# Roestlab/diffusion-deconvolution-dia-msms-data

Measured on AMD Instinct MI355X. Metric: MS2 windows/s (train step: zero_grad + train_step + backward + clip 10 + AdamW), higher is better.
Workload: dtype f32; 1 GPU; BASELINE configs[1]: default UNet1d (dim 4, mults 1,2,2,3,3,4,4; 128,847 params), synthetic MS2+MS1 windows 400 RT x 64 m/z, batch 32 per GPU, fp32; global_batch=32, parallelism=dp1

## Files before the change

diffusion-deconvolution-dia-msms-data_amd/csrc/dq_kernels.h:

```cpp
#pragma once
#include <hip/hip_runtime.h>
#include <cstdint>

namespace dq {

constexpr int MSE_MAX_BLOCKS = 1024;

int launch_q_sample(const float* alpha_bars, const float* x0, const int64_t* t, const float* noise, float* x_t, int B,
                    int64_t per_sample, int normalize, hipStream_t s);
int launch_sample_finish(const float* x, const float* ms2_cond, float* out_x, float* out_noise, int64_t n, int normalize,
                         hipStream_t s);
int launch_mse_fwd_bwd(const float* eps, const float* noise, float* loss_out, float* grad_out, float* partials, int64_t n,
                       hipStream_t s, const float* lw = nullptr, const int64_t* t = nullptr, int64_t per_sample = 0, float tm = 1.f,
                       float ta = 0.f, int* defer_sum = nullptr);
int launch_sum_partials(const float* partials, int count, float scale, float* out, hipStream_t s);
int launch_ms1_loss(const float* out, const float* x_t, const float* ms1, float cm, float ca, const float* lw, const int64_t* t, float w,
                    int B, int RT, int MZ, float* grad, float* loss_out, float* scratch, hipStream_t s);
constexpr int MSE_PW_SLICE = 8192;
int64_t mse_per_window_scratch_bytes(int B, int64_t per);
int launch_mse_per_window(const float* out, const float* target, float tm, float ta, const float* lw, const int64_t* t, float* per_window,
                          float* loss_out, void* scratch, int64_t scratch_bytes, int B, int64_t per, hipStream_t s);
int launch_axpy(float* dst, const float* src, int64_t n, hipStream_t s);
int launch_zero(float* dst, int64_t n, hipStream_t s);
int launch_copy(float* dst, const float* src, int64_t n, hipStream_t s);
// ... 247 lines not shown
struct ConvBwdWg {
  const float* dy = nullptr;
  const float* in = nullptr;
  const float* w = nullptr;
  float* din = nullptr; int accumulate = 0;
  float* part = nullptr; int64_t part_floats = 0;
  float* dparams = nullptr;
  int C = 0, pre = 0, cp = 0, rows = 0, n = 0, rows_per_sample = 1;
  int tiles_ps = 0, tpb = 0, nv = 0;
};
bool conv_wg_usable(int C, int pre, int cp, int n, int rows_per_sample);
int64_t conv_wg_part_floats(int C, int pre, int cp, int B, int rows_per_sample, int n);
int launch_conv_bwd_wg(const ConvBwdWg& a, hipStream_t s, ResWgReduce* red_out);
inline PartReduce res_part_reduce(const float* gpart, int gx, int B, int C, float* dg2, float* dg1, float* dss, int ss_stride) {
  PartReduce r;
  r.part = gpart; r.B = B; r.gx = gx; r.nv = 4 * C; r.nseg = 2;
  r.seg_start[0] = 0; r.seg_len[0] = C; r.seg_dst[0] = dg2;
  r.seg_start[1] = C; r.seg_len[1] = C; r.seg_dst[1] = dg1;
  r.s0 = 2 * C; r.sn = 2 * C; r.sdst = dss; r.sstride = ss_stride;
  return r;
}

int launch_rmsnorm_fwd(const float* x, const float* g, float* y, int C, int rows, int n, hipStream_t s);

int launch_fold(const float* in, float* out, int B, int RT, int cn, int to_mid, int add, hipStream_t s, int pitch = 0);

int launch_prep_inputs(const float* x, const float* cond, const float* ms1, const float* ss, int ss_stride, int ss_off, float cm,
                       float ca, float* cat0, float* ms1n, int B, int RT, int MZ, hipStream_t s);
int launch_ms1_norm(const float* ms1, float cm, float ca, float* ms1n, int64_t n, hipStream_t s);
constexpr int MS1_MAX_CHANNELS = 4096;
constexpr int MS1_FWD_TP = 8, MS1_FWD_WAVES = 4;
constexpr int MS1_WG_T = 64, MS1_WG_MAX_PARTS = 256;
struct Ms1FeatFwd {
  const float* ms1 = nullptr;
  const float* w = nullptr; const float* bias = nullptr;
  float cm = 1.f, ca = 0.f;
  float* ms1n_out = nullptr;
  float* u_out = nullptr;
  float* a_out = nullptr;
  int B = 0, RT = 0, M1 = 0;
};
int launch_ms1_feat_fwd(const Ms1FeatFwd& a, hipStream_t s);
struct Ms1FeatWgrad {
  const float* ms1n = nullptr; const float* du = nullptr;
  float* dw = nullptr; float* dbias = nullptr;
  float* part = nullptr; int64_t part_floats = 0;
  int B = 0, RT = 0, M1 = 0;
};
int ms1_feat_wgrad_parts(int B, int RT, int M1);
int64_t ms1_feat_wgrad_part_floats(int B, int RT, int M1);
int launch_ms1_feat_wgrad(const Ms1FeatWgrad& a, hipStream_t s);
int launch_prep_inputs_bwd(const float* dcat0, const float* cond, float cm, float ca, float* dss, int ss_stride, int ss_off, int B,
                           int RT, int MZ, float* part, int64_t part_floats, hipStream_t s);

int launch_im2col3(const float* x, float* xcol, int B, int C, int RT, int P, hipStream_t s);
int launch_col2im3(const float* dxcol, float* dx, int B, int C, int RT, int P, int accumulate, hipStream_t s);
int launch_repitch(float* dst, int dpitch, const float* src, int spitch, int64_t rows, int n, hipStream_t s);
int launch_zero_pads(float* x, int64_t rows, int RT, int P, hipStream_t s);
int launch_wnorm_fwd(const float* u, const float* g, const float* ss, int ss_stride, int act, const float* res, float* y, int B, int C,
                     int RT, int P, hipStream_t s);
int launch_wnorm_bwd(const float* u, const float* dy, const float* g, const float* ss, int ss_stride, int act, float* du, float* dg,
                     float* dss, float* dbias, float* scratch, int B, int C, int RT, int P, hipStream_t s);
int launch_rowsum(const float* x, int64_t rows, int RT, int P, float* out, hipStream_t s);
int launch_sum_b(const float* part, int B, int C, float* dst, hipStream_t s);


struct LinAttn {
  const float* x = nullptr; float* y = nullptr;
  const float* w_qkv = nullptr; const float* w_out = nullptr; const float* b_out = nullptr;
  const float* g_pre = nullptr; const float* g_out = nullptr;
  int C = 0, rows = 0, n = 0;
  float* ypre = nullptr;
  const float* prep = nullptr;
};
inline bool la_short_row(int n) { return n <= 64 && (n & (n - 1)) == 0; }
enum LaFwdForm { LA_FWD_LONG, LA_FWD_SMALL, LA_FWD_ROWS, LA_FWD_REG };
LaFwdForm la_fwd_form(const LinAttn& a);
int launch_linattn_fwd(const LinAttn& a, hipStream_t s);
bool la_small_usable(int C, int n);
int la_small_min_rows();
int launch_la_small_fwd(const LinAttn& a, hipStream_t s);
struct LinAttnBwd;
bool la_rows_bwd_usable(int C, int n);
int la_rows_bwd_min_rows();
bool la_rows_fwd_usable(int C, int n);
int launch_la_rows_fwd(const LinAttn& a, hipStream_t s);
int launch_la_rows_bwd(const LinAttnBwd& a, int max_slots, int* slots_out, hipStream_t s);
constexpr int LA_PREP_BOUNDED = 1024 + 4096;
constexpr int LA_PREP_BF16 = 1024 + 4096 + 8;
constexpr int LA_PREP_SMALL = 1024 + 4096 + 8 + 6144;
constexpr int LA_ROWS_LANE_FLOATS = 36;
constexpr int LA_PREP_ROWS = 1024 + 4096 + 8 + 6144 + 6144;
constexpr int LA_PREP_FLOATS = LA_PREP_ROWS + 4 * 64 * LA_ROWS_LANE_FLOATS;
struct LaPrepItem { const float* w_qkv; const float* w_out; int C; float* prep; const float* g_pre; };
constexpr int LA_PREP_MAX = 16;
struct PrepCopy { const float* src; float* dst; int n; };
constexpr int PREP_COPY_MAX = 4;
int launch_linattn_prepare(const LaPrepItem* items, int count, hipStream_t s, const PrepCopy* copies = nullptr, int n_copies = 0);
struct LinAttnBwd {
  LinAttn f;
  const float* dy = nullptr; float* dx = nullptr;
  int dx_store = 0;
  const float* ypre = nullptr;
  float* dyp = nullptr; float* dxh = nullptr;
  float* part = nullptr; int64_t part_floats = 0;
  int defer_reduce = 0; int* waves_out = nullptr;
// ... 33 lines not shown
```

diffusion-deconvolution-dia-msms-data_amd/csrc/dq_unet.hip:

```cpp
#include "dq_dev.h"
#include "dq_tfm.h"
#include "dq_ops.h"
#include "dq_options.h"
#include "../../include/dq_hip.h"

#include <algorithm>
#include <functional>
#include <cmath>
#include <cstdlib>
#include <cstring>
#include <vector>

namespace dq {

void layout_arena(const Plan& p, int B, int RT, Arena& a) {
  int64_t zero_total = 0;
  for (int pass = 0; pass < 2; ++pass) {
  a = Arena();
  a.B = B; a.RT = RT;
  int64_t off = 0, off_nz = zero_total;
  auto take = [&](int64_t n) { int64_t o = off; off += (n + 63) / 64 * 64; return o; };
  auto take_nz = [&](int64_t n) { int64_t o = off_nz; off_nz += (n + 63) / 64 * 64; return o; };
  const int64_t R = (int64_t)B * RT;
  auto res = [&](int rows_per_sample, int cin, int c, int n, bool zero_out = false) {
// ... 735 lines not shown
      DQ_TRY(tiny_bwd_run(c, tiny_bwd_desc(c, true, lp.tb_up_w), true));
    } else {
      DQ_TRY(la_bwd(c, l.la, b, c.w(b.r1.out), c.g(b.la), c.g(b.r1.out), R, l.n, lp.prep_ok ? L + ui : -1));
      DQ_TRY(res_bwd(c, l.r1, b.r1, c.w(b.r0.out), c.g(b.r0.out), cx, c.w(a.downs[lv].r0.out), c.g(a.downs[lv].r0.out), cs, R, l.n, RT, 1, 1));
      DQ_TRY(res_bwd(c, l.r0, b.r0, c.w(in_off), c.g(in_off), cx, c.w(a.downs[lv].la), c.g(a.downs[lv].la), cs, R, l.n, RT, 1, 1));
    }
    if (side_flush_here(lv)) DQ_TRY(side_flush(c));
  }
  if (p.wide_mid) {
    DQ_TRY(mid_backward_wide(c, rope));
  } else {
    if (!lp.use_tb_up) DQ_TRY(launch_fold(c.g(a.mid_back), c.g(a.mid2.out), B, RT, p.mid_c, 1, 1, c.s));
    DQ_TRY(mid_backward(c, rope, grad_x != nullptr, lp.prep_ok));
    if (!lp.use_tb_dn) DQ_TRY(launch_fold(c.g(a.mid_in), c.g(a.downs[L - 1].rs), B, RT, p.mid_c, 0, 0, c.s));
  }
  auto ms1_bwd = [&p, &a, B, RT](const Ctx& cc) -> int {
    DQ_TRY(conv_plain_bwd(cc, p.ms1_c1, CONV_S1, cc.w(a.ms1_a), cc.g(a.ms1f), cc.g(a.ms1_a), B, RT, RT, 0));
    BlockBwd gb;
    gb.u = cc.w(a.ms1_u); gb.dy = cc.g(a.ms1_a); gb.du = cc.g(a.ms1_u); gb.C = p.cond_dim; gb.rows = B; gb.n = RT; gb.rows_per_sample = 1;
    gb.act = ACT_GELU;
    DQ_TRY(launch_block_bwd(gb, cc.s));
    if (p.ms1_channels > 1) {
      Ms1FeatWgrad w;
      w.ms1n = cc.w(a.ms1n); w.du = cc.g(a.ms1_u); w.dw = cc.dprm(p.ms1_c0.w); w.dbias = cc.dprm(p.ms1_c0.b);
      w.part = cc.w(a.ms1_wpart); w.part_floats = a.ms1_wpart_floats; w.B = B; w.RT = RT; w.M1 = p.ms1_channels;
      return launch_ms1_feat_wgrad(w, cc.s);
    }
    return conv_plain_bwd(cc, p.ms1_c0, CONV_S1, cc.w(a.ms1n), cc.g(a.ms1_u), nullptr, B, RT, RT, 0);
  };
  DQ_TRY(on_side(c, tail_fork_enabled(), ms1_bwd));
  for (int lv = L - 1; lv >= 0; --lv) {
    const LevelP& l = p.downs[lv];
    const LevelBuf& b = a.downs[lv];
    const int C = l.r0.cin;
    const int64_t in_off = lv == 0 ? a.h0 : a.downs[lv - 1].rs;
    if (lv == L - 1 && lp.use_tb_dn) {
      DQ_TRY(tiny_bwd_run(c, tiny_bwd_desc(c, false, false), false));
      if (side_flush_here(lv)) DQ_TRY(side_flush(c));
      continue;
    }
    if (!(lv == L - 2 && lp.use_tb_dn))
      DQ_TRY(resample_bwd(c, l.resample, l.last ? LEVEL_PRE_S1 : LEVEL_PRE_DOWN, b, l.n, l.n_next, 1));
    if (lv == 0) DQ_TRY(side_flush(c));
    DQ_TRY(la_bwd(c, l.la, b, c.w(b.r1.out), c.g(b.la), c.g(b.r1.out), R, l.n, lp.prep_ok ? lv : -1));
    DQ_TRY(res_bwd(c, l.r1, b.r1, c.w(b.r0.out), c.g(b.r0.out), C, nullptr, nullptr, 0, R, l.n, RT));
    if (lv == 0) DQ_TRY(side_flush(c));
    DQ_TRY(res_bwd(c, l.r0, b.r0, c.w(in_off), c.g(in_off), C, nullptr, nullptr, 0, R, l.n, RT, lv > 0 ? 1 : 0, 0));
    if (lv == 2 && p.mz <= 64) {
      DQ_TRY(la_flush_side(c));
      DQ_TRY(wg_to_side());
    }
    if (side_flush_here(lv)) DQ_TRY(side_flush(c));
  }
  auto init_bwd = [&p, &a, init_cond, cm, ca, B, RT, R](const Ctx& cc) -> int {
    DQ_TRY(conv_plain_bwd(cc, p.init_conv, CONV_S1, cc.w(a.cat0), cc.g(a.h0), cc.g(a.cat0), R, p.mz, p.mz, 0));
    return launch_prep_inputs_bwd(cc.g(a.cat0), init_cond, cm, ca, cc.g(a.ss), p.ss_total, p.ss_init, B, RT, p.mz, cc.w(a.bb_part),
                                  a.bb_part_floats, cc.s);
  };
  const bool tail_swap = !DQ_DEV_FLAG("DQ_NO_TAIL_SWAP", '1');
  if (side_open(c, tail_swap && !grad_x && tail_fork_enabled())) {
    DQ_TRY(side_flush(c));
    hipEvent_t ev_ss = nullptr;
    if (c.owner->side_used) DQ_TRY(side_mark(c, &ev_ss));
    DQ_TRY(conv_plain_bwd(c, p.init_conv, CONV_S1, c.w(a.cat0), c.g(a.h0), nullptr, R, p.mz, p.mz, 0));
    DQ_TRY(la_flush_side(c));
    DQ_TRY(side_flush(c));
    DQ_TRY(conv_plain_bwd(c, p.init_conv, CONV_S1, c.w(a.cat0), c.g(a.h0), c.g(a.cat0), R, p.mz, p.mz, 0, -1, false));
    if (ev_ss) DQ_HIP_OK(hipStreamWaitEvent(c.s, ev_ss, 0));
    DQ_TRY(launch_prep_inputs_bwd(c.g(a.cat0), init_cond, cm, ca, c.g(a.ss), p.ss_total, p.ss_init, B, RT, p.mz, c.w(a.bb_part), a.bb_part_floats,
                                  c.s));
    DQ_TRY(la_flush(c));
    DQ_TRY(res_wg_reduce_all(wg_items, c.s));
    DQ_TRY(launch_time_embed_bwd(p, dt, c.P, c.dP, c.w(a.tbuf), c.g(a.ss), B, c.s));
    return join_side(c);
  }
  DQ_TRY(on_side(c, !grad_x && tail_fork_enabled(), init_bwd));
  if (grad_x) {
    DQ_HIP_OK(hipMemcpy2DAsync(grad_x, sizeof(float) * p.mz, c.g(a.cat0) + p.mz, sizeof(float) * 2 * p.mz, sizeof(float) * p.mz, R,
                               hipMemcpyDeviceToDevice, c.s));
  }
  DQ_TRY(bwd_close(c, queues));
  return launch_time_embed_bwd(p, dt, c.P, c.dP, c.w(a.tbuf), c.g(a.ss), B, c.s);
}

int unet_sample_prologue(const Ctx& c, const float* ms1, float cm, float ca, const float* rope, bool* ran) {
  const Plan& p = c.p;
  const Arena& a = c.ar;
  *ran = false;
  if (p.wide_mid) return 0;
  const LevelPlan lp = level_plan(p, a, c.B, c.RT, false, false);
  DQ_TRY(unet_prepare(c, lp, c.s));
  DQ_TRY(ms1_features(c, ms1, cm, ca, true, c.s));
  DQ_TRY(conv_plain_fwd(c, proj(p.k_w, HID, p.cond_dim), CONV_S1, c.w(a.ms1f), c.w(a.kk), c.B, c.RT, c.RT, lp.prep_ok ? 1 : -1));
  if (rope) DQ_TRY(launch_rope(c.w(a.kk), rope, c.B, (int64_t)HID * c.RT, c.RT, 1.f, c.s));
  *ran = true;
  return 0;
}

int ensure_arena(dq_plan* plan, int B, int RT) {
  if (plan->arena.B != B || plan->arena.RT != RT) layout_arena(plan->plan, B, RT, plan->arena);
  if (!plan->dev.ss_w_off) {
    const Plan& p = plan->plan;
    std::vector<int64_t> woff(p.ss_total), boff(p.ss_total);
    for (const auto& l : p.ss_lins)
      for (int r = 0; r < l.rows; ++r) {
        woff[l.ss_off + r] = l.w + (int64_t)r * p.time_dim;
        boff[l.ss_off + r] = l.b + r;
      }
    DQ_HIP_OK(hipMalloc(&plan->dev.ss_w_off, sizeof(int64_t) * p.ss_total));
    DQ_HIP_OK(hipMalloc(&plan->dev.ss_b_off, sizeof(int64_t) * p.ss_total));
    DQ_HIP_OK(hipMemcpy(plan->dev.ss_w_off, woff.data(), sizeof(int64_t) * p.ss_total, hipMemcpyHostToDevice));
    DQ_HIP_OK(hipMemcpy(plan->dev.ss_b_off, boff.data(), sizeof(int64_t) * p.ss_total, hipMemcpyHostToDevice));
  }
  return 0;
}

}

using namespace dq;

extern "C" {

int dq_debug_level_plan(dq_plan* plan, int B, int RT, int save, int twin, int32_t* out, int cap) {
// ... 163 lines not shown
```

diffusion-deconvolution-dia-msms-data_amd/csrc/k_conv.hip:

```cpp
#include "dq_common.h"
#include "dq_kernels.h"
#include <cstdlib>

namespace dq {

template <int MODE, int K>
__device__ __forceinline__ int tap_pos(int p, int k, int n_in) {
  if (MODE == CONV_S1) {
    const int q = p + k - (K - 1) / 2;
    return (q >= 0 && q < n_in) ? q : -1;
  } else if (MODE == CONV_DOWN) {
    const int q = 2 * p + k - 1;
    return (q >= 0 && q < n_in) ? q : -1;
  } else {
    const int j = p + k - 1;
    return (j >= 0 && j < 2 * n_in) ? (j >> 1) : -1;
  }
}

template <int COUT, int K, int MODE>
__global__ void __launch_bounds__(256) k_conv_fwd(ConvFwd a) {
  const int64_t item = blockIdx.x * (int64_t)blockDim.x + threadIdx.x;
  const int64_t total = (int64_t)a.rows * a.n_out;
  const int co_base = blockIdx.y * COUT;
// ... 950 lines not shown
    const int b = (int)(i / ((int64_t)RT * cn));
    const int64_t src = ((int64_t)b * cn + c) * P + rt;
    out[i] = add ? out[i] + in[src] : in[src];
  }
}

int launch_fold(const float* in, float* out, int B, int RT, int cn, int to_mid, int add, hipStream_t s, int pitch) {
  const int P = pitch > 0 ? pitch : RT;
  const int64_t total = (int64_t)B * (to_mid ? P : RT) * cn;
  if (total == 0) return 0;
  hipLaunchKernelGGL(k_fold, dim3(cdiv(total, 256)), dim3(256), 0, s, in, out, B, RT, cn, to_mid, add, P);
  DQ_LAUNCH_CHECK();
  return 0;
}

__global__ void __launch_bounds__(256) k_prep_inputs(const float* __restrict__ x, const float* __restrict__ cond,
                                                     const float* __restrict__ ms1, const float* __restrict__ ss, int ss_stride,
                                                     int ss_off, float cm, float ca, float* __restrict__ cat0,
                                                     float* __restrict__ ms1n, int B, int RT, int MZ) {
  const int64_t i = blockIdx.x * (int64_t)blockDim.x + threadIdx.x;
  const int64_t total = (int64_t)B * RT * MZ;
  if (ms1n && i < (int64_t)B * RT) ms1n[i] = fmaf(ms1[i], cm, ca);
  if (i >= total) return;
  const int mz = (int)(i % MZ);
  const int64_t row = i / MZ;
  const int b = (int)(row / RT);
  const float sc = ss[(int64_t)b * ss_stride + ss_off], sh = ss[(int64_t)b * ss_stride + ss_off + 1];
  const float cn = fmaf(cond[i], cm, ca);
  cat0[(row * 2 + 0) * MZ + mz] = cn * (sc + 1.0f) + sh;
  cat0[(row * 2 + 1) * MZ + mz] = x[i];
}

int launch_prep_inputs(const float* x, const float* cond, const float* ms1, const float* ss, int ss_stride, int ss_off, float cm,
                       float ca, float* cat0, float* ms1n, int B, int RT, int MZ, hipStream_t s) {
  const int64_t total = (int64_t)B * RT * MZ;
  if (total == 0) return 0;
  hipLaunchKernelGGL(k_prep_inputs, dim3(cdiv(total, 256)), dim3(256), 0, s, x, cond, ms1, ss, ss_stride, ss_off, cm, ca, cat0,
                     ms1n, B, RT, MZ);
  DQ_LAUNCH_CHECK();
  return 0;
}

__global__ void __launch_bounds__(256) k_ms1_norm(const float* __restrict__ ms1, float cm, float ca, float* __restrict__ ms1n, int64_t n) {
  const int64_t i = blockIdx.x * (int64_t)blockDim.x + threadIdx.x;
  if (i < n) ms1n[i] = fmaf(ms1[i], cm, ca);
}
int launch_ms1_norm(const float* ms1, float cm, float ca, float* ms1n, int64_t n, hipStream_t s) {
  if (n == 0) return 0;
  hipLaunchKernelGGL(k_ms1_norm, dim3(cdiv(n, 256)), dim3(256), 0, s, ms1, cm, ca, ms1n, n);
  DQ_LAUNCH_CHECK();
  return 0;
}

__global__ void __launch_bounds__(256) k_prep_inputs_bwd(const float* __restrict__ dcat0, const float* __restrict__ cond, float cm,
                                                         float ca, float* __restrict__ part, int RT, int MZ) {
  const int b = blockIdx.y;
  const int64_t per = (int64_t)RT * MZ;
  float dsc = 0.f, dsh = 0.f;
  for (int64_t it = blockIdx.x * (int64_t)blockDim.x + threadIdx.x; it < per; it += (int64_t)gridDim.x * blockDim.x) {
    const int mz = (int)(it % MZ);
    const int64_t row = (int64_t)b * RT + it / MZ;
    const float d = dcat0[(row * 2 + 0) * MZ + mz];
    dsh += d;
    dsc = fmaf(d, fmaf(cond[(int64_t)b * per + it], cm, ca), dsc);
  }
  __shared__ float red[4][2];
  dsc = wave_sum(dsc);
  dsh = wave_sum(dsh);
  if ((threadIdx.x & 63) == 0) { red[threadIdx.x >> 6][0] = dsc; red[threadIdx.x >> 6][1] = dsh; }
  __syncthreads();
  if (threadIdx.x < 2)
    part[((int64_t)b * gridDim.x + blockIdx.x) * 2 + threadIdx.x] =
        (red[0][threadIdx.x] + red[1][threadIdx.x]) + (red[2][threadIdx.x] + red[3][threadIdx.x]);
}

int launch_prep_inputs_bwd(const float* dcat0, const float* cond, float cm, float ca, float* dss, int ss_stride, int ss_off, int B,
                           int RT, int MZ, float* part, int64_t part_floats, hipStream_t s) {
  const int64_t per = (int64_t)RT * MZ;
  if (per == 0 || B == 0) return 0;
  dim3 grid(std::max(1, std::min(32, cdiv(per, 1024))), B);
  DQ_REQUIRE(part && part_floats >= (int64_t)grid.x * B * 2, "prep_inputs_bwd: partial-sum slot missing or too small");
  hipLaunchKernelGGL(k_prep_inputs_bwd, grid, dim3(256), 0, s, dcat0, cond, cm, ca, part, RT, MZ);
  DQ_LAUNCH_CHECK();
  PartReduce r;
  r.part = part; r.B = B; r.gx = (int)grid.x; r.nv = 2; r.s0 = 0; r.sn = 2; r.sdst = dss + ss_off; r.sstride = ss_stride;
  return launch_part_reduce(r, s);
}

}
```

diffusion-deconvolution-dia-msms-data_amd/csrc/k_res_wg.hip:

```cpp
#include "dq_common.h"
#include "dq_kernels.h"
#include "k_res_common.h"
#include "dq_probe.h"
#include <algorithm>

namespace dq {

namespace {

typedef float f32x4 __attribute__((ext_vector_type(4)));
__device__ __forceinline__ f32x4 mfma4(float a, float b, f32x4 c) { return __builtin_amdgcn_mfma_f32_4x4x1f32(a, b, c, 0, 0, 0); }

__device__ __forceinline__ float lane_m1(float v) { return __int_as_float(__builtin_amdgcn_mov_dpp(__float_as_int(v), 0x138, 0xF, 0xF, true)); }
__device__ __forceinline__ float lane_p1(float v) { return __int_as_float(__builtin_amdgcn_mov_dpp(__float_as_int(v), 0x130, 0xF, 0xF, true)); }
constexpr int pad4(int x) { return (x + 3) / 4 * 4; }

constexpr int TILE = 256;
constexpr int RUN = 16;

template <int C>
struct Img {
  static constexpr int ST = C == 4 ? 4 : 12;
  static constexpr int FLOATS = (TILE + 2) * ST + ((TILE + 2) / RUN + 1) * 4;
  __device__ static __forceinline__ int at(int q) { return q * ST + (q >> 4) * 4; }
};
template <int ST>
__device__ __forceinline__ constexpr int run_off(int s) { return s * ST + (s == RUN - 1 ? 4 : 0); }


}

template <int C, bool WR>
__global__ void __launch_bounds__(256, 2) k_res_bwd_wg(ResBwdWg a) {
  using I = Img<C>;
  constexpr int ST = I::ST, CQ = C / 4;
  extern __shared__ __attribute__((aligned(16))) float lds_all[];
  float* i_du2 = lds_all;
  float* i_du1 = i_du2 + I::FLOATS;
  float* i_a1 = i_du1 + I::FLOATS;
  float* i_xa = i_a1 + I::FLOATS;
  float* i_xb = i_xa + I::FLOATS;
  float* i_do = i_xb + (WR ? I::FLOATS : 4);
  float (*red)[4 * C] = reinterpret_cast<float (*)[4 * C]>(i_do + (WR ? I::FLOATS : 4));
  constexpr int GI = WR ? 2 * CQ : CQ;
  constexpr int JT2 = C * CQ * 3, JT1 = C * GI * 3, JTR = WR ? C * GI : 0;
  constexpr int OT1 = pad4(JT2), OTR = OT1 + pad4(JT1), JTT = OTR + pad4(JTR);
  float* wl = reinterpret_cast<float*>(red) + 4 * 4 * C;
  float* prm = wl + JTT * 4;
  const int cin = a.cinA + a.cinB;
  DQ_PSTAMP(100000 + C * 10 + (WR ? 1 : 0), 0);
  for (int idx = threadIdx.x; idx < JTT * 4; idx += 256) {
    const int j = (idx >> 4) * 4 + (idx & 3), l4 = (idx >> 2) & 3;
    float v = 0.f;
    if (j < JT2) {
      const int k = j % 3, gg = (j / 3) % CQ, co = j / (3 * CQ);
      v = a.w2[(co * C + 4 * gg + l4) * 3 + k];
    } else if (j >= OT1 && j < OT1 + JT1) {
      const int jj = j - OT1, k = jj % 3, gi = (jj / 3) % GI, co = jj / (3 * GI), ci = 4 * gi + l4;
      if (ci < cin) v = a.w1[(co * cin + ci) * 3 + k];
    } else if (WR && j >= OTR && j < OTR + JTR) {
      const int jj = j - OTR, gi = jj % GI, co = jj / GI, ci = 4 * gi + l4;
      if (ci < cin) v = a.wr[co * cin + ci];
    }
    wl[idx] = v;
  }
  for (int i = threadIdx.x; i < 4 * C; i += 256) {
    const int what = i / C, c = i % C;
    const float* ssp = a.ss + (int64_t)blockIdx.y * a.ss_stride;
    prm[i] = what == 0 ? a.g2[c] : what == 1 ? a.g1[c] : what == 2 ? ssp[c] : ssp[C + c];
  }
  __syncthreads();
  DQ_PSTAMP(100000 + C * 10 + (WR ? 1 : 0), 1);
  const int b = blockIdx.y, n = a.n;
  const int per_sample = a.rows_per_sample * n;
  const int tid = threadIdx.x, lane = tid & 63;
  const int wv = __builtin_amdgcn_readfirstlane(tid >> 6);
  const int q = tid + 1;
  const int blk = lane >> 2, li = lane & 3;
  const int lb = I::at(blk * RUN + 1) + li;
  const bool n8 = n == 8;
  const bool zl = ((blk * RUN) % n) == 0;
  const bool zr = ((blk * RUN + RUN) % n) == 0;
  const int cinq = cin >> 2;
  const int g = C == 8 ? (wv & 1) : 0, hs = C == 8 ? (wv >> 1) : wv;
  const bool doW2 = C == 8 ? true : wv == 0;
  const int hW2 = C == 8 ? hs : 0;
  const bool doB2 = C == 8 ? hs == 0 : wv == 0;
  const bool doWr = WR && (C == 8 ? true : wv == 1);
  const int hr0 = C == 8 ? 2 * hs : 0, hr1 = C == 8 ? 2 * hs + 1 : 1;
  const bool doBr = WR && (C == 8 ? hs == 0 : wv == 1);
  const bool doW1 = C == 8 ? true : (wv == 2 || (WR && wv == 3));
  const int h10 = C == 8 ? (WR ? 2 * hs : hs) : (wv == 3 ? 1 : 0);
  const int h11 = (C == 8 && WR) ? 2 * hs + 1 : -1;
  const bool doB1 = C == 8 ? hs == 0 : wv == 2;
  const bool v_r0 = doWr && hr0 < cinq, v_r1 = doWr && hr1 < cinq;
  const bool v_10 = doW1 && h10 < cinq, v_11 = doW1 && h11 >= 0 && h11 < cinq;
  auto ximg = [&](int h) -> const float* { return (h < CQ || !WR ? i_xa + 4 * (h < CQ ? h : 0) : i_xb + 4 * (h - CQ)) + lb; };

  f32x4 aW2[1][3], aWr[2], aW1[2][3], aB2 = {0.f, 0.f, 0.f, 0.f}, aBr = aB2, aB1 = aB2;
#pragma unroll
  for (int h = 0; h < 1; ++h)
#pragma unroll
    for (int k = 0; k < 3; ++k) aW2[h][k] = aB2;
#pragma unroll
  for (int h = 0; h < 2; ++h) {
#pragma unroll
    for (int k = 0; k < 3; ++k) aW1[h][k] = aB2;
    aWr[h] = aB2;
  }
  float dg2[C], dg1[C], dsc[C], dsh[C];
#pragma unroll
  for (int c = 0; c < C; ++c) dg2[c] = dg1[c] = dsc[c] = dsh[c] = 0.f;
  const float sqC = sqrtf((float)C);
  const float* wlane = wl + li * 4;
  auto wop = [&](int j) -> float { return wlane[(j >> 2) * 16 + (j & 3)]; };

  const int tile_end = min(a.tiles_ps, ((int)blockIdx.x + 1) * a.tpb);
#pragma unroll 1
  for (int tile = blockIdx.x * a.tpb; tile < tile_end; ++tile) {
    const int it = tile * TILE + tid;
    const bool live = it < per_sample;
    const int itc = live ? it : per_sample - 1;
    const int row = b * a.rows_per_sample + itc / n, p = itc % n;
    const unsigned boA = (((unsigned)row * C) * (unsigned)n + (unsigned)p) * 4u;
    const unsigned boB = (((unsigned)row * (unsigned)a.cinB) * (unsigned)n + (unsigned)p) * 4u;
    auto ld = [&](const float* base, int c, unsigned boff) -> float {
      return *reinterpret_cast<const float*>(reinterpret_cast<const char*>(base + (size_t)c * n) + boff);
    };
    auto st = [&](float* base, int c, unsigned boff, float v) {
      *reinterpret_cast<float*>(reinterpret_cast<char*>(base + (size_t)c * n) + boff) = v;
    };
    const bool hasL = live && p > 0, hasR = live && p + 1 < n;
    float dout[C], d[C], u[C], u1v[C], xa[C], xb[WR ? C : 1];
#pragma unroll
    for (int c = 0; c < C; ++c) {
      dout[c] = ld(a.dout, c, boA);
      u[c] = ld(a.u2, c, boA);
      u1v[c] = ld(a.u1, c, boA);
      xa[c] = ld(a.inA, c, boA);
    }
    if constexpr (WR) {
#pragma unroll
      for (int c = 0; c < C; ++c) xb[c] = c < a.cinB ? ld(a.inB, c, boB) : 0.f;
    }
#pragma unroll
    for (int c = 0; c < C; ++c) { dout[c] = live ? dout[c] : 0.f; d[c] = dout[c]; }
    norm_act_bwd<C, false>(u, d, prm, nullptr, dg2, nullptr, nullptr);
    float a1v[C];
    {
      float ssq = 0.f;
#pragma unroll
      for (int c = 0; c < C; ++c) ssq = fmaf(u1v[c], u1v[c], ssq);
      const float inv = rms_inv(ssq, sqC);
#pragma unroll
      for (int c = 0; c < C; ++c) a1v[c] = silu_f(fmaf(u1v[c] * inv * prm[C + c], prm[2 * C + c] + 1.0f, prm[3 * C + c]));
    }
    DQ_PSTAMP(100000 + C * 10 + (WR ? 1 : 0), 2);
    __syncthreads();
    {
      const int o = I::at(q);
#pragma unroll
      for (int c4 = 0; c4 < CQ; ++c4) {
        const int c = 4 * c4;
        *reinterpret_cast<float4*>(i_du2 + o + c) = live ? make_float4(d[c], d[c + 1], d[c + 2], d[c + 3]) : make_float4(0.f, 0.f, 0.f, 0.f);
        *reinterpret_cast<float4*>(i_a1 + o + c) = make_float4(a1v[c], a1v[c + 1], a1v[c + 2], a1v[c + 3]);
        *reinterpret_cast<float4*>(i_xa + o + c) = make_float4(xa[c], xa[c + 1], xa[c + 2], xa[c + 3]);
        if constexpr (WR) {
          *reinterpret_cast<float4*>(i_xb + o + c) = make_float4(xb[c], xb[c + 1], xb[c + 2], xb[c + 3]);
          *reinterpret_cast<float4*>(i_do + o + c) = make_float4(dout[c], dout[c + 1], dout[c + 2], dout[c + 3]);
        }
      }
    }
    __syncthreads();
    DQ_PSTAMP(100000 + C * 10 + (WR ? 1 : 0), 3);
    if (doW2) {
      const float* A = i_du2 + lb + 4 * g;
      const float* Bp = i_a1 + lb + 4 * hW2;
      float bprev = zl ? 0.f : Bp[-ST], bcur = Bp[0];
#pragma unroll
      for (int s = 0; s < RUN; ++s) {
        const float av = A[run_off<ST>(s)];
        float bnext = s + 1 < RUN ? Bp[run_off<ST>(s + 1 < RUN ? s + 1 : s)] : (zr ? 0.f : Bp[RUN * ST + 4]);
        float b0 = bprev, b2 = bnext;
        if (s == 8) b0 = n8 ? 0.f : b0;
        if (s == 7) b2 = n8 ? 0.f : b2;
        aW2[0][0] = mfma4(av, b0, aW2[0][0]);
        aW2[0][1] = mfma4(av, bcur, aW2[0][1]);
        aW2[0][2] = mfma4(av, b2, aW2[0][2]);
        aB2 = mfma4(av, 1.f, aB2);
        bprev = bcur; bcur = bnext;
      }
    }
    if constexpr (WR) {
     if (doWr) {
      const float* A = i_do + lb + 4 * g;
      const float* X0 = ximg(hr0);
// ... 75 lines not shown
    }
    DQ_PSTAMP(100000 + C * 10 + (WR ? 1 : 0), 8);
    if (a.dA || a.dB) {
#pragma unroll
      for (int pass = 0; pass < (WR ? 2 : 1); ++pass) {
        f32x4 acc[CQ][3], ar[CQ];
#pragma unroll
        for (int q4 = 0; q4 < CQ; ++q4) {
#pragma unroll
          for (int k = 0; k < 3; ++k) acc[q4][k] = f32x4{0.f, 0.f, 0.f, 0.f};
          ar[q4] = f32x4{0.f, 0.f, 0.f, 0.f};
        }
#pragma unroll
        for (int co = 0; co < C; ++co) {
          const float dc = live ? da1[co] : 0.f;
          const float tp = lane_p1(dc), tm = lane_m1(dc);
          const float dr = hasR ? tp : 0.f, dl = hasL ? tm : 0.f;
#pragma unroll
          for (int q4 = 0; q4 < CQ; ++q4) {
            const int gi = pass * CQ + q4;
            const int j = OT1 + (co * GI + gi) * 3;
            acc[q4][0] = mfma4(wop(j + 0), dr, acc[q4][0]);
            acc[q4][1] = mfma4(wop(j + 1), dc, acc[q4][1]);
            acc[q4][2] = mfma4(wop(j + 2), dl, acc[q4][2]);
            if constexpr (WR) ar[q4] = mfma4(wop(OTR + co * GI + gi), dout[co], ar[q4]);
          }
        }
        if (pass == 0) DQ_PSTAMP(100000 + C * 10 + (WR ? 1 : 0), 11);
        float v[C];
#pragma unroll
        for (int q4 = 0; q4 < CQ; ++q4)
#pragma unroll
          for (int i = 0; i < 4; ++i) v[4 * q4 + i] = (acc[q4][0][i] + acc[q4][1][i]) + (acc[q4][2][i] + (WR ? ar[q4][i] : dout[4 * q4 + i]));
        if (pass == 0) {
          if (live && a.dA) {
            float oldv[C];
#pragma unroll
            for (int c = 0; c < C; ++c) oldv[c] = 0.f;
            if (!a.dA_store) {
#pragma unroll
              for (int c = 0; c < C; ++c) oldv[c] = ld(a.dA, c, boA);
            }
            DQ_PSTAMP(100000 + C * 10 + (WR ? 1 : 0), 12);
#pragma unroll
            for (int c = 0; c < C; ++c) st(a.dA, c, boA, oldv[c] + v[c]);
          }
        } else {
          if (live && a.dB) {
            float oldv[C];
#pragma unroll
            for (int c = 0; c < C; ++c) oldv[c] = 0.f;
            if (!a.dB_store) {
#pragma unroll
              for (int c = 0; c < C; ++c) oldv[c] = c < a.cinB ? ld(a.dB, c, boB) : 0.f;
            }
#pragma unroll
            for (int c = 0; c < C; ++c)
              if (c < a.cinB) st(a.dB, c, boB, oldv[c] + v[c]);
          }
        }
      }
    }
    DQ_PSTAMP(100000 + C * 10 + (WR ? 1 : 0), 9);
  }

  float* part = a.part + ((int64_t)blockIdx.y * gridDim.x + blockIdx.x) * a.nv;
  const int oC1W = 0, oC1B = C * cin * 3, oG1 = oC1B + C, oC2W = oG1 + C, oC2B = oC2W + C * C * 3, oG2 = oC2B + C, oRW = oG2 + C,
            oRB = oRW + C * cin, nglob = WR ? oRB + C : oRW;
  auto put_w = [&](f32x4 acc, int base, int h, int kdim, int k, int ld) {
    const f32x4 t = blocks_sum(acc);
    if (lane < 4) {
#pragma unroll
      for (int i = 0; i < 4; ++i) part[base + ((4 * g + i) * ld + 4 * h + lane) * kdim + k] = t[i];
    }
  };
  auto put_b = [&](f32x4 acc, int base) {
    const f32x4 t = blocks_sum(acc);
    if (lane == 0) {
#pragma unroll
      for (int i = 0; i < 4; ++i) part[base + 4 * g + i] = t[i];
    }
  };
  if (doW2) {
#pragma unroll
    for (int k = 0; k < 3; ++k) put_w(aW2[0][k], oC2W, hW2, 3, k, C);
  }
  if (doB2) put_b(aB2, oC2B);
  if (v_r0) put_w(aWr[0], oRW, hr0, 1, 0, cin);
  if (v_r1) put_w(aWr[1], oRW, hr1, 1, 0, cin);
  if (doBr) put_b(aBr, oRB);
  if (v_10) {
#pragma unroll
    for (int k = 0; k < 3; ++k) put_w(aW1[0][k], oC1W, h10, 3, k, cin);
  }
  if (v_11) {
#pragma unroll
    for (int k = 0; k < 3; ++k) put_w(aW1[1][k], oC1W, h11, 3, k, cin);
  }
  if (doB1) put_b(aB1, oC1B);
#pragma unroll
  for (int c = 0; c < C; ++c) {
    const float s0 = wave_sum(dg2[c]), s1 = wave_sum(dg1[c]), s2 = wave_sum(dsc[c]), s3 = wave_sum(dsh[c]);
    if (lane == 0) { red[wv][c] = s0; red[wv][C + c] = s1; red[wv][2 * C + c] = s2; red[wv][3 * C + c] = s3; }
  }
  __syncthreads();
  for (int i = tid; i < 4 * C; i += 256) {
    const float v = (red[0][i] + red[1][i]) + (red[2][i] + red[3][i]);
    const int what = i / C, c = i % C;
    part[(what == 0 ? oG2 : what == 1 ? oG1 : what == 2 ? nglob : nglob + C) + c] = v;
  }
  DQ_PSTAMP(100000 + C * 10 + (WR ? 1 : 0), 10);
}

__global__ void __launch_bounds__(256) k_res_wg_reduce(ResWgReduceMulti m) {
  const ResWgReduce& r = m.it[blockIdx.y];
  const int twoC = 2 * r.C;
  const int nelem = r.nglob + r.B * twoC;
// ... 22 lines not shown
    if (k < cnt) s0 += src[(int64_t)k * r.nv];
  }
  red[gq][el] = s0 + s1;
  __syncthreads();
  if (gq == 0 && e < nelem) {
    float s = 0.f;
#pragma unroll
    for (int k = 0; k < 16; ++k) s += red[k][el];
    if (e < r.nglob) r.dst[e] += s;
    else r.dss[(int64_t)((e - r.nglob) / twoC) * r.ss_stride + (e - r.nglob) % twoC] += s;
  }
}

bool res_wg_usable(int n, int C, int cinA, int cinB, int rows_per_sample) {
  if (!(C == 4 || C == 8)) return false;
  return n >= 8 && n <= 64 && (n & (n - 1)) == 0 && rows_per_sample > 1 && cinA == C && (cinB == 0 || (cinB % 4 == 0 && cinB <= C));
}

template <int C, bool WR>
static size_t res_wg_lds_bytes() {
  constexpr int CQ = C / 4, GI = WR ? 2 * CQ : CQ;
  constexpr int JT2 = C * CQ * 3, JT1 = C * GI * 3, JTR = WR ? C * GI : 0;
  constexpr int JTT = pad4(JT2) + pad4(JT1) + pad4(JTR);
  return sizeof(float) * ((size_t)(WR ? 6 : 4) * Img<C>::FLOATS + (WR ? 0 : 8) + 16 * C + (size_t)JTT * 4 + 4 * C);
}

void res_wg_grid(int B, int rows_per_sample, int n, int* tiles_ps, int* tpb, int* gx) {
  *tiles_ps = cdiv((int64_t)rows_per_sample * n, TILE);
  const int64_t total = (int64_t)*tiles_ps * B;
  *tpb = (int)std::max<int64_t>(1, (total + 1023) / 1024);
  *gx = cdiv(*tiles_ps, *tpb);
}
int res_wg_nv(int C, int cin, bool wr) { return C * cin * 3 + C + C + C * C * 3 + C + C + (wr ? C * cin + C : 0) + 2 * C; }
int64_t res_wg_part_floats(int C, int cin, bool wr, int B, int rows_per_sample, int n) {
  int tiles_ps, tpb, gx;
  res_wg_grid(B, rows_per_sample, n, &tiles_ps, &tpb, &gx);
  return (int64_t)gx * B * res_wg_nv(C, cin, wr);
}

int launch_res_bwd_wg(const ResBwdWg& a_in, hipStream_t s, ResWgReduce* red_out) {
  ResBwdWg a = a_in;
  DQ_REQUIRE(res_wg_usable(a.n, a.C, a.cinA, a.cinB, a.rows_per_sample), "res_bwd_wg: unsupported shape");
  DQ_REQUIRE(a.rows % a.rows_per_sample == 0, "res_bwd_wg: rows must be a multiple of rows_per_sample");
  DQ_REQUIRE((int64_t)a.rows * a.C * a.n * 4 < (1ll << 32), "res_bwd_wg: tensors of 4 GB or more are not built (32-bit byte offsets)");
  DQ_REQUIRE(a.wr || a.cinB == 0, "res_bwd_wg: identity residual needs C input channels");
  DQ_REQUIRE(a.dout && a.u1 && a.u2 && a.inA && (a.cinB == 0 || a.inB) && a.w1 && a.w2 && a.g1 && a.g2 && a.ss && a.part,
             "res_bwd_wg: missing operand");
  const int B = a.rows / a.rows_per_sample;
  int gx;
  res_wg_grid(B, a.rows_per_sample, a.n, &a.tiles_ps, &a.tpb, &gx);
  const bool wr = a.wr != nullptr;
  const void* fn = nullptr;
  size_t lds = 0;
#define DQ_WGK(CC, WW) if (a.C == CC && wr == WW) { fn = (const void*)k_res_bwd_wg<CC, WW>; lds = res_wg_lds_bytes<CC, WW>(); }
  DQ_WGK(4, true) DQ_WGK(4, false) DQ_WGK(8, true) DQ_WGK(8, false)
#undef DQ_WGK
  DQ_REQUIRE(fn && lds <= 160 * 1024, "res_bwd_wg: no kernel for this shape");
  {
    static int occ[2][2] = {{0, 0}, {0, 0}};
    int& o = occ[a.C / 4 - 1][wr];
    if (!o) {
      if (lds > 48 * 1024) DQ_HIP_OK(hipFuncSetAttribute(fn, hipFuncAttributeMaxDynamicSharedMemorySize, (int)lds));
      int nb = 0;
      DQ_HIP_OK(hipOccupancyMaxActiveBlocksPerMultiprocessor(&nb, fn, 256, lds));
      o = std::max(1, std::min(nb, 6));
    }
    int dev = 0;
    hipDeviceProp_t pr;
    static const int cus = (hipGetDevice(&dev) == hipSuccess && hipGetDeviceProperties(&pr, dev) == hipSuccess) ? pr.multiProcessorCount : 256;
    const int64_t resident = (int64_t)o * cus, total = (int64_t)a.tiles_ps * B;
    a.tpb = std::max(a.tpb, (int)((total + resident - 1) / resident));
    while (a.tpb < a.tiles_ps && (int64_t)cdiv(a.tiles_ps, a.tpb) * B > resident) ++a.tpb;
    gx = cdiv(a.tiles_ps, a.tpb);
  }
  a.nv = res_wg_nv(a.C, a.cinA + a.cinB, wr);
  DQ_REQUIRE(a.part_floats >= (int64_t)gx * B * a.nv, "res_bwd_wg: slot scratch too small");
  dim3 grid(gx, B), block(256);
#define DQ_WGL(CC, WW) if (a.C == CC && wr == WW) hipLaunchKernelGGL((k_res_bwd_wg<CC, WW>), grid, block, lds, s, a);
  DQ_WGL(4, true) DQ_WGL(4, false) DQ_WGL(8, true) DQ_WGL(8, false)
#undef DQ_WGL
  DQ_LAUNCH_CHECK();
  if (red_out) {
    ResWgReduce r;
    r.part = a.part; r.B = B; r.gx = gx; r.nv = a.nv; r.nglob = a.nv - 2 * a.C; r.C = a.C;
    r.dst = a.dparams; r.dss = a.dss; r.ss_stride = a.ss_stride;
    *red_out = r;
  }
  return 0;
}

int launch_res_wg_reduce(const ResWgReduce* items, int count, hipStream_t s) {
  if (count == 0) return 0;
  DQ_REQUIRE(count <= RES_WG_REDUCE_MAX, "res_wg_reduce: too many items");
  ResWgReduceMulti m;
  int nmax = 1;
  for (int i = 0; i < count; ++i) {
    m.it[i] = items[i];
    DQ_REQUIRE(items[i].part && items[i].dst && items[i].dss, "res_wg_reduce: missing operand");
    nmax = std::max(nmax, items[i].nglob + items[i].B * 2 * items[i].C);
  }
  hipLaunchKernelGGL(k_res_wg_reduce, dim3(cdiv(nmax, 16), count), dim3(256), 0, s, m);
  DQ_LAUNCH_CHECK();
  return 0;
}

}
```

Before: 10220 windows/s.

## Fuse init-conv input-grad into cond-scale reduction; specialize res wgrad kernel on row length

Adds a kernel that computes the init convolution's input gradient on the fly inside the conditioning scale/shift reduction, so the dcat0 gradient tensor is no longer written and reread. Separately templates the residual weight-gradient kernel on the row length N, which turns the div/mod into compile-time shifts, precomputes byte offsets, splits full and tail tiles, and raises launch-bounds occupancy for C=4. These are unrelated ideas bundled together. The cost is more template instantiations and a recomputed convolution whose inner loop over output channels is less parallel.

Result: no change. 10160 windows/s (-0.5%).

```diff
diff --git a/diffusion-deconvolution-dia-msms-data_amd/csrc/dq_kernels.h b/diffusion-deconvolution-dia-msms-data_amd/csrc/dq_kernels.h
--- a/diffusion-deconvolution-dia-msms-data_amd/csrc/dq_kernels.h
+++ b/diffusion-deconvolution-dia-msms-data_amd/csrc/dq_kernels.h
@@ -323,6 +323,9 @@
 int launch_ms1_feat_wgrad(const Ms1FeatWgrad& a, hipStream_t s);
 int launch_prep_inputs_bwd(const float* dcat0, const float* cond, float cm, float ca, float* dss, int ss_stride, int ss_off, int B,
                            int RT, int MZ, float* part, int64_t part_floats, hipStream_t s);
+bool init_cond_bwd_usable(int cout, int K, int mode);
+int launch_init_cond_bwd(const float* dh0, const float* w, int cout, int cin, const float* cond, float cm, float ca, float* dss,
+                         int ss_stride, int ss_off, int B, int RT, int MZ, float* part, int64_t part_floats, hipStream_t s);
 
 int launch_im2col3(const float* x, float* xcol, int B, int C, int RT, int P, hipStream_t s);
 int launch_col2im3(const float* dxcol, float* dx, int B, int C, int RT, int P, int accumulate, hipStream_t s);
diff --git a/diffusion-deconvolution-dia-msms-data_amd/csrc/dq_unet.hip b/diffusion-deconvolution-dia-msms-data_amd/csrc/dq_unet.hip
--- a/diffusion-deconvolution-dia-msms-data_amd/csrc/dq_unet.hip
+++ b/diffusion-deconvolution-dia-msms-data_amd/csrc/dq_unet.hip
@@ -811,10 +811,18 @@
     }
     if (side_flush_here(lv)) DQ_TRY(side_flush(c));
   }
-  auto init_bwd = [&p, &a, init_cond, cm, ca, B, RT, R](const Ctx& cc) -> int {
-    DQ_TRY(conv_plain_bwd(cc, p.init_conv, CONV_S1, cc.w(a.cat0), cc.g(a.h0), cc.g(a.cat0), R, p.mz, p.mz, 0));
+  const bool fuse_cond = !grad_x && init_cond_bwd_usable(p.init_conv.cout, p.init_conv.k, CONV_S1);
+  auto cond_bwd = [&p, &a, init_cond, cm, ca, B, RT, R, fuse_cond](const Ctx& cc) -> int {
+    if (fuse_cond)
+      return launch_init_cond_bwd(cc.g(a.h0), cc.prm(p.init_conv.w), p.init_conv.cout, p.init_conv.cin, init_cond, cm, ca, cc.g(a.ss),
+                                  p.ss_total, p.ss_init, B, RT, p.mz, cc.w(a.bb_part), a.bb_part_floats, cc.s);
+    DQ_TRY(conv_plain_bwd(cc, p.init_conv, CONV_S1, cc.w(a.cat0), cc.g(a.h0), cc.g(a.cat0), R, p.mz, p.mz, 0, -1, false));
     return launch_prep_inputs_bwd(cc.g(a.cat0), init_cond, cm, ca, cc.g(a.ss), p.ss_total, p.ss_init, B, RT, p.mz, cc.w(a.bb_part),
                                   a.bb_part_floats, cc.s);
+  };
+  auto init_bwd = [&p, &a, R, cond_bwd](const Ctx& cc) -> int {
+    DQ_TRY(conv_plain_bwd(cc, p.init_conv, CONV_S1, cc.w(a.cat0), cc.g(a.h0), nullptr, R, p.mz, p.mz, 0));
+    return cond_bwd(cc);
   };
   const bool tail_swap = !DQ_DEV_FLAG("DQ_NO_TAIL_SWAP", '1');
   if (side_open(c, tail_swap && !grad_x && tail_fork_enabled())) {
@@ -824,10 +832,8 @@
     DQ_TRY(conv_plain_bwd(c, p.init_conv, CONV_S1, c.w(a.cat0), c.g(a.h0), nullptr, R, p.mz, p.mz, 0));
     DQ_TRY(la_flush_side(c));
     DQ_TRY(side_flush(c));
-    DQ_TRY(conv_plain_bwd(c, p.init_conv, CONV_S1, c.w(a.cat0), c.g(a.h0), c.g(a.cat0), R, p.mz, p.mz, 0, -1, false));
     if (ev_ss) DQ_HIP_OK(hipStreamWaitEvent(c.s, ev_ss, 0));
-    DQ_TRY(launch_prep_inputs_bwd(c.g(a.cat0), init_cond, cm, ca, c.g(a.ss), p.ss_total, p.ss_init, B, RT, p.mz, c.w(a.bb_part), a.bb_part_floats,
-                                  c.s));
+    DQ_TRY(cond_bwd(c));
     DQ_TRY(la_flush(c));
     DQ_TRY(res_wg_reduce_all(wg_items, c.s));
     DQ_TRY(launch_time_embed_bwd(p, dt, c.P, c.dP, c.w(a.tbuf), c.g(a.ss), B, c.s));
diff --git a/diffusion-deconvolution-dia-msms-data_amd/csrc/k_conv.hip b/diffusion-deconvolution-dia-msms-data_amd/csrc/k_conv.hip
--- a/diffusion-deconvolution-dia-msms-data_amd/csrc/k_conv.hip
+++ b/diffusion-deconvolution-dia-msms-data_amd/csrc/k_conv.hip
@@ -1026,6 +1026,17 @@
   return 0;
 }
 
+__device__ __forceinline__ void prep_inputs_flush(float dsc, float dsh, float* __restrict__ part) {
+  __shared__ float red[4][2];
+  dsc = wave_sum(dsc);
+  dsh = wave_sum(dsh);
+  if ((threadIdx.x & 63) == 0) { red[threadIdx.x >> 6][0] = dsc; red[threadIdx.x >> 6][1] = dsh; }
+  __syncthreads();
+  if (threadIdx.x < 2)
+    part[((int64_t)blockIdx.y * gridDim.x + blockIdx.x) * 2 + threadIdx.x] =
+        (red[0][threadIdx.x] + red[1][threadIdx.x]) + (red[2][threadIdx.x] + red[3][threadIdx.x]);
+}
+
 __global__ void __launch_bounds__(256) k_prep_inputs_bwd(const float* __restrict__ dcat0, const float* __restrict__ cond, float cm,
                                                          float ca, float* __restrict__ part, int RT, int MZ) {
   const int b = blockIdx.y;
@@ -1038,27 +1049,73 @@
     dsh += d;
     dsc = fmaf(d, fmaf(cond[(int64_t)b * per + it], cm, ca), dsc);
   }
-  __shared__ float red[4][2];
-  dsc = wave_sum(dsc);
-  dsh = wave_sum(dsh);
-  if ((threadIdx.x & 63) == 0) { red[threadIdx.x >> 6][0] = dsc; red[threadIdx.x >> 6][1] = dsh; }
+  prep_inputs_flush(dsc, dsh, part);
+}
+
+constexpr int INIT_TAIL_K = 7, INIT_TAIL_WMAX = 1024;
+__global__ void __launch_bounds__(256) k_init_cond_bwd(const float* __restrict__ du, const float* __restrict__ w, int cout, int cin,
+                                                       const float* __restrict__ cond, float cm, float ca, float* __restrict__ part,
+                                                       int RT, int MZ) {
+  constexpr int K = INIT_TAIL_K;
+  __shared__ float wsh[INIT_TAIL_WMAX];
+  for (int i = threadIdx.x; i < cout * K; i += 256) wsh[i] = w[(int64_t)(i / K) * cin * K + i % K];
   __syncthreads();
-  if (threadIdx.x < 2)
-    part[((int64_t)b * gridDim.x + blockIdx.x) * 2 + threadIdx.x] =
-        (red[0][threadIdx.x] + red[1][threadIdx.x]) + (red[2][threadIdx.x] + red[3][threadIdx.x]);
+  const int b = blockIdx.y;
+  const int64_t per = (int64_t)RT * MZ;
+  float dsc = 0.f, dsh = 0.f;
+  for (int64_t it = blockIdx.x * (int64_t)blockDim.x + threadIdx.x; it < per; it += (int64_t)gridDim.x * blockDim.x) {
+    const int mz = (int)(it % MZ);
+    const int64_t row = (int64_t)b * RT + it / MZ;
+    float acc = 0.f;
+    for (int co = 0; co < cout; ++co) {
+      const float* dup = du + (row * cout + co) * MZ;
+      float dv[K];
+#pragma unroll
+      for (int k = 0; k < K; ++k) {
+        const int p = mz - k + (K - 1) / 2;
+        dv[k] = (p >= 0 && p < MZ) ? dup[p] : 0.f;
+      }
+#pragma unroll
+      for (int k = 0; k < K; ++k) acc = fmaf(wsh[co * K + k], dv[k], acc);
+    }
+    const float d = 0.f + acc;
+    dsh += d;
+    dsc = fmaf(d, fmaf(cond[(int64_t)b * per + it], cm, ca), dsc);
+  }
+  prep_inputs_flush(dsc, dsh, part);
+}
+
+namespace {
+dim3 prep_inputs_grid(int64_t per, int B) { return dim3(std::max(1, std::min(32, cdiv(per, 1024))), B); }
+int prep_inputs_reduce(float* part, int B, int gx, float* dss, int ss_stride, int ss_off, hipStream_t s) {
+  PartReduce r;
+  r.part = part; r.B = B; r.gx = gx; r.nv = 2; r.s0 = 0; r.sn = 2; r.sdst = dss + ss_off; r.sstride = ss_stride;
+  return launch_part_reduce(r, s);
+}
 }
 
 int launch_prep_inputs_bwd(const float* dcat0, const float* cond, float cm, float ca, float* dss, int ss_stride, int ss_off, int B,
                            int RT, int MZ, float* part, int64_t part_floats, hipStream_t s) {
   const int64_t per = (int64_t)RT * MZ;
   if (per == 0 || B == 0) return 0;
-  dim3 grid(std::max(1, std::min(32, cdiv(per, 1024))), B);
+  const dim3 grid = prep_inputs_grid(per, B);
   DQ_REQUIRE(part && part_floats >= (int64_t)grid.x * B * 2, "prep_inputs_bwd: partial-sum slot missing or too small");
   hipLaunchKernelGGL(k_prep_inputs_bwd, grid, dim3(256), 0, s, dcat0, cond, cm, ca, part, RT, MZ);
   DQ_LAUNCH_CHECK();
-  PartReduce r;
-  r.part = part; r.B = B; r.gx = (int)grid.x; r.nv = 2; r.s0 = 0; r.sn = 2; r.sdst = dss + ss_off; r.sstride = ss_stride;
-  return launch_part_reduce(r, s);
-}
-
-}
+  return prep_inputs_reduce(part, B, (int)grid.x, dss, ss_stride, ss_off, s);
+}
+
+bool init_cond_bwd_usable(int cout, int K, int mode) { return K == INIT_TAIL_K && mode == CONV_S1 && cout > 0 && cout * K <= INIT_TAIL_WMAX; }
+int launch_init_cond_bwd(const float* dh0, const float* w, int cout, int cin, const float* cond, float cm, float ca, float* dss,
+                         int ss_stride, int ss_off, int B, int RT, int MZ, float* part, int64_t part_floats, hipStream_t s) {
+  const int64_t per = (int64_t)RT * MZ;
+  if (per == 0 || B == 0) return 0;
+  DQ_REQUIRE(dh0 && w && cond && cin > 0 && init_cond_bwd_usable(cout, INIT_TAIL_K, CONV_S1), "init_cond_bwd: missing operand or unsupported conv");
+  const dim3 grid = prep_inputs_grid(per, B);
+  DQ_REQUIRE(part && part_floats >= (int64_t)grid.x * B * 2, "init_cond_bwd: partial-sum slot missing or too small");
+  hipLaunchKernelGGL(k_init_cond_bwd, grid, dim3(256), 0, s, dh0, w, cout, cin, cond, cm, ca, part, RT, MZ);
+  DQ_LAUNCH_CHECK();
+  return prep_inputs_reduce(part, B, (int)grid.x, dss, ss_stride, ss_off, s);
+}
+
+}
diff --git a/diffusion-deconvolution-dia-msms-data_amd/csrc/k_res_wg.hip b/diffusion-deconvolution-dia-msms-data_amd/csrc/k_res_wg.hip
--- a/diffusion-deconvolution-dia-msms-data_amd/csrc/k_res_wg.hip
+++ b/diffusion-deconvolution-dia-msms-data_amd/csrc/k_res_wg.hip
@@ -3,6 +3,7 @@
 #include "k_res_common.h"
 #include "dq_probe.h"
 #include <algorithm>
+#include <type_traits>
 
 namespace dq {
 
@@ -30,10 +31,12 @@
 
 }
 
-template <int C, bool WR>
-__global__ void __launch_bounds__(256, 2) k_res_bwd_wg(ResBwdWg a) {
+template <int C, bool WR, int N>
+__global__ void __launch_bounds__(256, (C == 4 && !(WR && N <= 16)) ? 4 : 2) k_res_bwd_wg(ResBwdWg a) {
+  static_assert(N == 8 || N == 16 || N == 32 || N == 64, "rows of 8, 16, 32 or 64 positions");
   using I = Img<C>;
   constexpr int ST = I::ST, CQ = C / 4;
+  constexpr int LOGN = N == 8 ? 3 : N == 16 ? 4 : N == 32 ? 5 : 6;
   extern __shared__ __attribute__((aligned(16))) float lds_all[];
   float* i_du2 = lds_all;
   float* i_du1 = i_du2 + I::FLOATS;
@@ -71,16 +74,24 @@
   }
   __syncthreads();
   DQ_PSTAMP(100000 + C * 10 + (WR ? 1 : 0), 1);
-  const int b = blockIdx.y, n = a.n;
-  const int per_sample = a.rows_per_sample * n;
+  const int b = blockIdx.y;
+  const int per_sample = a.rows_per_sample * N;
   const int tid = threadIdx.x, lane = tid & 63;
   const int wv = __builtin_amdgcn_readfirstlane(tid >> 6);
   const int q = tid + 1;
   const int blk = lane >> 2, li = lane & 3;
   const int lb = I::at(blk * RUN + 1) + li;
-  const bool n8 = n == 8;
-  const bool zl = ((blk * RUN) % n) == 0;
-  const bool zr = ((blk * RUN + RUN) % n) == 0;
+  constexpr bool n8 = N == 8;
+  const bool zl = ((blk * RUN) % N) == 0;
+  const bool zr = ((blk * RUN + RUN) % N) == 0;
+  auto inB_has = [&](int c) -> bool { return (c & ~3) < a.cinB; };
+  const int p = tid & (N - 1);
+  const bool hasLp = p > 0, hasRp = p + 1 < N;
+  const unsigned row0 = (unsigned)b * (unsigned)a.rows_per_sample;
+  const unsigned loA = ((row0 + (unsigned)(tid >> LOGN)) * (unsigned)(C * N) + (unsigned)p) * 4u;
+  const unsigned loB = ((row0 + (unsigned)(tid >> LOGN)) * (unsigned)a.cinB * (unsigned)N + (unsigned)p) * 4u;
+  const unsigned endA = ((row0 + (unsigned)a.rows_per_sample - 1u) * (unsigned)(C * N) + (unsigned)(N - 1)) * 4u;
+  const unsigned endB = ((row0 + (unsigned)a.rows_per_sample - 1u) * (unsigned)a.cinB * (unsigned)N + (unsigned)(N - 1)) * 4u;
   const int cinq = cin >> 2;
   const int g = C == 8 ? (wv & 1) : 0, hs = C == 8 ? (wv >> 1) : wv;
   const bool doW2 = C == 8 ? true : wv == 0;
@@ -115,22 +126,18 @@
   const float* wlane = wl + li * 4;
   auto wop = [&](int j) -> float { return wlane[(j >> 2) * 16 + (j & 3)]; };
 
-  const int tile_end = min(a.tiles_ps, ((int)blockIdx.x + 1) * a.tpb);
-#pragma unroll 1
-  for (int tile = blockIdx.x * a.tpb; tile < tile_end; ++tile) {
-    const int it = tile * TILE + tid;
-    const bool live = it < per_sample;
-    const int itc = live ? it : per_sample - 1;
-    const int row = b * a.rows_per_sample + itc / n, p = itc % n;
-    const unsigned boA = (((unsigned)row * C) * (unsigned)n + (unsigned)p) * 4u;
-    const unsigned boB = (((unsigned)row * (unsigned)a.cinB) * (unsigned)n + (unsigned)p) * 4u;
+  auto do_tile = [&](auto full, const int tile) {
+    constexpr bool FULL = decltype(full)::value;
+    const bool live = FULL ? true : tile * TILE + tid < per_sample;
+    const unsigned tA = loA + (unsigned)tile * (unsigned)(TILE * C * 4), tB = loB + (unsigned)tile * ((unsigned)a.cinB * (unsigned)(TILE * 4));
+    const unsigned boA = live ? tA : endA, boB = live ? tB : endB;
     auto ld = [&](const float* base, int c, unsigned boff) -> float {
-      return *reinterpret_cast<const float*>(reinterpret_cast<const char*>(base + (size_t)c * n) + boff);
+      return *reinterpret_cast<const float*>(reinterpret_cast<const char*>(base) + boff + c * (N * 4));
     };
     auto st = [&](float* base, int c, unsigned boff, float v) {
-      *reinterpret_cast<float*>(reinterpret_cast<char*>(base + (size_t)c * n) + boff) = v;
+      *reinterpret_cast<float*>(reinterpret_cast<char*>(base) + boff + c * (N * 4)) = v;
     };
-    const bool hasL = live && p > 0, hasR = live && p + 1 < n;
+    const bool hasL = live && hasLp, hasR = live && hasRp;
     float dout[C], d[C], u[C], u1v[C], xa[C], xb[WR ? C : 1];
 #pragma unroll
     for (int c = 0; c < C; ++c) {
@@ -141,7 +148,7 @@
     }
     if constexpr (WR) {
 #pragma unroll
-      for (int c = 0; c < C; ++c) xb[c] = c < a.cinB ? ld(a.inB, c, boB) : 0.f;
+      for (int c = 0; c < C; ++c) xb[c] = inB_has(c) ? ld(a.inB, c, boB) : 0.f;
     }
 #pragma unroll
     for (int c = 0; c < C; ++c) { dout[c] = live ? dout[c] : 0.f; d[c] = dout[c]; }
@@ -323,17 +330,22 @@
             for (int c = 0; c < C; ++c) oldv[c] = 0.f;
             if (!a.dB_store) {
 #pragma unroll
-              for (int c = 0; c < C; ++c) oldv[c] = c < a.cinB ? ld(a.dB, c, boB) : 0.f;
+              for (int c = 0; c < C; ++c) oldv[c] = inB_has(c) ? ld(a.dB, c, boB) : 0.f;
             }
 #pragma unroll
             for (int c = 0; c < C; ++c)
-              if (c < a.cinB) st(a.dB, c, boB, oldv[c] + v[c]);
+              if (inB_has(c)) st(a.dB, c, boB, oldv[c] + v[c]);
           }
         }
       }
     }
     DQ_PSTAMP(100000 + C * 10 + (WR ? 1 : 0), 9);
-  }
+  };
+  const int tile_end = min(a.tiles_ps, ((int)blockIdx.x + 1) * a.tpb);
+  const int full_end = min(tile_end, per_sample / TILE);
+#pragma unroll 1
+  for (int tile = blockIdx.x * a.tpb; tile < full_end; ++tile) do_tile(std::true_type{}, tile);
+  if (full_end < tile_end) do_tile(std::false_type{}, full_end);
 
   float* part = a.part + ((int64_t)blockIdx.y * gridDim.x + blockIdx.x) * a.nv;
   const int oC1W = 0, oC1B = C * cin * 3, oG1 = oC1B + C, oC2W = oG1 + C, oC2B = oC2W + C * C * 3, oG2 = oC2B + C, oRW = oG2 + C,
@@ -462,13 +474,15 @@
   const bool wr = a.wr != nullptr;
   const void* fn = nullptr;
   size_t lds = 0;
-#define DQ_WGK(CC, WW) if (a.C == CC && wr == WW) { fn = (const void*)k_res_bwd_wg<CC, WW>; lds = res_wg_lds_bytes<CC, WW>(); }
-  DQ_WGK(4, true) DQ_WGK(4, false) DQ_WGK(8, true) DQ_WGK(8, false)
+#define DQ_WGK(CC, WW, NN) if (a.C == CC && wr == WW && a.n == NN) { fn = (const void*)k_res_bwd_wg<CC, WW, NN>; lds = res_wg_lds_bytes<CC, WW>(); }
+#define DQ_WGN(CC, WW) DQ_WGK(CC, WW, 8) DQ_WGK(CC, WW, 16) DQ_WGK(CC, WW, 32) DQ_WGK(CC, WW, 64)
+  DQ_WGN(4, true) DQ_WGN(4, false) DQ_WGN(8, true) DQ_WGN(8, false)
+#undef DQ_WGN
 #undef DQ_WGK
   DQ_REQUIRE(fn && lds <= 160 * 1024, "res_bwd_wg: no kernel for this shape");
   {
-    static int occ[2][2] = {{0, 0}, {0, 0}};
-    int& o = occ[a.C / 4 - 1][wr];
+    static int occ[2][2][4] = {};
+    int& o = occ[a.C / 4 - 1][wr][a.n == 8 ? 0 : a.n == 16 ? 1 : a.n == 32 ? 2 : 3];
     if (!o) {
       if (lds > 48 * 1024) DQ_HIP_OK(hipFuncSetAttribute(fn, hipFuncAttributeMaxDynamicSharedMemorySize, (int)lds));
       int nb = 0;
@@ -486,8 +500,10 @@
   a.nv = res_wg_nv(a.C, a.cinA + a.cinB, wr);
   DQ_REQUIRE(a.part_floats >= (int64_t)gx * B * a.nv, "res_bwd_wg: slot scratch too small");
   dim3 grid(gx, B), block(256);
-#define DQ_WGL(CC, WW) if (a.C == CC && wr == WW) hipLaunchKernelGGL((k_res_bwd_wg<CC, WW>), grid, block, lds, s, a);
-  DQ_WGL(4, true) DQ_WGL(4, false) DQ_WGL(8, true) DQ_WGL(8, false)
+#define DQ_WGL(CC, WW, NN) if (a.C == CC && wr == WW && a.n == NN) hipLaunchKernelGGL((k_res_bwd_wg<CC, WW, NN>), grid, block, lds, s, a);
+#define DQ_WGN(CC, WW) DQ_WGL(CC, WW, 8) DQ_WGL(CC, WW, 16) DQ_WGL(CC, WW, 32) DQ_WGL(CC, WW, 64)
+  DQ_WGN(4, true) DQ_WGN(4, false) DQ_WGN(8, true) DQ_WGN(8, false)
+#undef DQ_WGN
 #undef DQ_WGL
   DQ_LAUNCH_CHECK();
   if (red_out) {
```
